# DLR-RM/AugmentedAutoencoder

Hardware: AMD Instinct MI355X
Metric: crops/sec (encode+codebook-NN), 128x128x3 vs 92232x128 codebook, 1/8 GPU (higher is better)
Workload: dtype f32; 1 GPU; configs[1]: single object per GPU, batch=256 uint8 128x128x3 crops, HIP 4-conv encoder -> 128-d + cosine-NN vs 92232x128 fp32 codebook, top-1; batch_per_gpu=256, codebook_rows=92232, latent=128, parallelism=single GPU

## Files before the change

### augmentedautoencoder_amd/csrc/aae_abi_impl.h

```cpp
#pragma once

extern "C" {

int aae_abi_version(void) { return AAE_ABI_VERSION; }
const char* aae_last_error(void) { return aae_host::g_last_error.c_str(); }

int aae_encoder_create(const aae_encoder_desc* d, const void* const* hw, int n_weights, aae_encoder** out) {
    using namespace aae_host;
    if (!d || !hw || !out) return fail(AAE_ERR_INVALID, "aae_encoder_create: null argument");
    if (d->num_layers < 1 || d->num_layers > AAE_MAX_LAYERS)
        return fail(AAE_ERR_INVALID, "num_layers %d outside [1,%d]", d->num_layers, AAE_MAX_LAYERS);
    if (d->in_h < 1 || d->in_w < 1 || d->in_c < 1 || d->kernel_size < 1 || d->latent_size < 1)
        return fail(AAE_ERR_INVALID, "non-positive shape in encoder desc");
    const int per_layer = d->batch_norm ? 6 : 2;
    if (n_weights != d->num_layers * per_layer + 2)
        return fail(AAE_ERR_INVALID, "expected %d weight arrays, got %d", d->num_layers * per_layer + 2, n_weights);
    for (int i = 0; i < n_weights; ++i)
        if (!hw[i]) return fail(AAE_ERR_INVALID, "weight array %d is null", i);

    aae_encoder* enc = new aae_encoder();
    enc->desc = *d;
    auto bail = [&](int rc) { aae_encoder_destroy(enc); return rc; };

    {
// ... 251 lines not shown
        if (value < -8 || value > 12) return fail(AAE_ERR_INVALID, "x3h_act_shift %d outside [-8, 12]", value);
        enc->x3h_act_shift = value;
    } else if (!strcmp(name, "winograd")) {
        if (value != 0) {
            bool any = false;
            for (const Layer& L : enc->layers) any = any || L.wino_geom >= 0;
            if (!any) return fail(AAE_ERR_UNSUPPORTED, "winograd: no layer is eligible (5 x 5 stride-2 'SAME' layers behind the first one with 32 | Cin, 64 | Cout and 16 | Ho, Wo or an 8 x 8 output)");
        }
        if (value < 0 || value > 2) return fail(AAE_ERR_INVALID, "winograd %d: 0 = direct kernels, 1 = one launch per layer, 2 = one launch per polyphase component", value);
#ifndef AAE_EXPERIMENTS
        if (value == 2) return fail(AAE_ERR_UNSUPPORTED, "option 'winograd' = 2 (one launch per polyphase component: measured slower) is a kernel variant of the experiments build (-DAAE_EXPERIMENTS)");
#endif
        enc->winograd = value;
    } else if (!strcmp(name, "winograd_wide")) {
        enc->winograd_wide = value ? 1 : 0;
    } else if (!strcmp(name, "winograd_min_batch")) {
        enc->winograd_min_batch = value < 1 ? 1 : value;
    } else if (!strcmp(name, "winograd_min_fill_pct")) {
        enc->winograd_min_fill_pct = value < 1 ? 1 : (value > 100 ? 100 : value);
    } else if (!strcmp(name, "winograd_min_blocks")) {
        enc->winograd_min_blocks = value < 0 ? 0 : value;
    } else if (!strcmp(name, "multi_mid_group")) {
        enc->multi_mid_group = value ? 1 : 0;
    } else if (!strcmp(name, "multi_split_items")) {
        enc->multi_split_items = value ? 1 : 0;
    } else if (!strcmp(name, "multi_group_winograd")) {
        enc->multi_group_winograd = value ? 1 : 0;
    } else if (!strcmp(name, "multi_mid_scan")) {
        enc->multi_mid_scan = value ? 1 : 0;
    } else if (!strcmp(name, "multi_mid_ragged")) {
// ... 458 lines not shown
```

### augmentedautoencoder_amd/csrc/aae_encoder_launch.h

```cpp
#pragma once

namespace aae_host {

struct Timer {
    bool on = false;
    hipStream_t stream = nullptr;
    std::vector<hipEvent_t> ev;
    int mark() {
        if (!on) return AAE_OK;
        hipEvent_t e;
        AAE_HIP_TRY(hipEventCreate(&e));
        ev.push_back(e);
        AAE_HIP_TRY(hipEventRecord(e, stream));
        return AAE_OK;
    }
};

static int launch_igemm(aae_encoder* enc, const Layer& L, const float* x, int M, float* out, float* partial,
                        hipStream_t stream, Timer& tm, const char* name, int tag = 0) {
    aae::ConvIgemmArgs a;
    a.x = x; a.wp = L.wp; a.bias = L.bias; a.bn_scale = L.bn_scale; a.bn_shift = L.bn_shift;
    a.H = L.H; a.W = L.W; a.Cin = L.Cin; a.Ho = L.Ho; a.Wo = L.Wo; a.Cout = L.Cout; a.CoutPad = L.CoutPad;
    a.KS = L.KS; a.S = L.S; a.pt = L.pt; a.pl = L.pl; a.M = M; a.relu = L.relu; a.stagger = enc->igemm_stagger;
    const unsigned long long x_bytes = (unsigned long long)(M / (L.Ho * L.Wo)) * L.H * L.W * L.Cin * sizeof(float);
// ... 520 lines not shown
            if (L.wino_geom == 0) launch_wino_phase<0>(a, eh, ew, grid, stream);
            else launch_wino_phase<1>(a, eh, ew, grid, stream);
            const int taps = (eh ? 3 : 2) * (ew ? 3 : 2), points = ((eh ? 3 : 2) + 1) * ((ew ? 3 : 2) + 1);
            snprintf(label, sizeof(label), "%s:conv_wino_f32 phase %d%d (%d taps as %d products per 2x2 outputs) M=%d N=%d C=%d", name, eh, ew, taps, points,
                     B * L.Ho * L.Wo, L.Cout, L.Cin);
            note_kernel({label, 2.0 * tiles * points * (double)L.Cin * (double)L.Cout});
            AAE_HIP_TRY(hipGetLastError());
            if (int rc = tm.mark()) return rc;
        }
        return AAE_OK;
    }
#endif
    aae::ConvWinoLayerArgs p;
    p.c = a;
    for (int i = 0; i < 4; ++i) p.U4[i] = L.wino[i];
    wino_layer_launch(L.wino_geom, enc->winograd_wide, grid, stream, p);
    snprintf(label, sizeof(label), "%s:conv_wino_f32 layer (25 taps as 49 products per 2x2 outputs) M=%d N=%d C=%d", name, B * L.Ho * L.Wo, L.Cout, L.Cin);
    note_kernel({label, 2.0 * tiles * 49.0 * (double)L.Cin * (double)L.Cout});
    AAE_HIP_TRY(hipGetLastError());
    return tm.mark();
}

static bool winograd_rule(const aae_encoder* enc, const Layer& L, int B);
static bool runs_winograd(const aae_encoder* enc, const Layer& L, int B) { return L.wino[0] && winograd_rule(enc, L, B); }
static bool wants_winograd_weights(const aae_encoder* enc, int B) {
    for (const Layer& L : enc->layers)
        if (L.kind == KIND_IGEMM && !L.wino[0] && winograd_rule(enc, L, B)) return true;
    return false;
}
static int ensure_winograd_weights(aae_encoder* enc) {
    std::lock_guard<std::mutex> lk(enc->wino_mu);
// ... 184 lines not shown
```

### augmentedautoencoder_amd/csrc/aae_host_types.h

```cpp
#pragma once

namespace aae_host {

static thread_local std::string g_last_error;

static int fail(int code, const char* fmt, ...) {
    char buf[512];
    va_list ap;
    va_start(ap, fmt);
    vsnprintf(buf, sizeof(buf), fmt, ap);
    va_end(ap);
    g_last_error = buf;
    return code;
}

#define AAE_HIP_TRY(expr)                                                                       \
    do {                                                                                        \
        hipError_t e__ = (expr);                                                                \
        if (e__ != hipSuccess)                                                                  \
            return aae_host::fail(AAE_ERR_RUNTIME, "%s failed: %s (%s:%d)", #expr,              \
                                  hipGetErrorString(e__), __FILE__, __LINE__);                  \
    } while (0)

static inline size_t align_up(size_t v, size_t a) { return (v + a - 1) / a * a; }
// ... 57 lines not shown
    std::mutex rec_mu;
    int splitk_min_base_blocks = 384;
    int splitk_target_blocks = 512;
    int reduce_small = 1;
    int precision = 0;
    int winograd = 1;
    int winograd_wide = 0;
    int winograd_min_batch = 8;
    int winograd_min_fill_pct = 56;
    int winograd_min_blocks = 0;
    int multi_mid_group = 1;
    int multi_split_items = 1;
    int multi_group_winograd = 1;
    int multi_mid_scan = 1;
    int multi_mid_ragged = 1;
    int winograd_xcd_cols = -1;
    int first_target_blocks = 512;
    int first_group_split_max_tiles = 128;
    int first_vec4 = 1;
    int first_max_tiles_per_block = 16;
    int igemm_breg_min_blocks = 768;
    int igemm_breg_wide = 1;
    int igemm_breg_wide_min_blocks = 512;
    int dense_gemv = 1;
    int dense_gemv_max_batch = 8;
    int igemm_breg = 1;
    int igemm_dma = 1;
    int x3h_wide_min_blocks = 0;
    int x3h_wide256 = 1;
    int x3h_wide256_min_blocks = 256;
// ... 57 lines not shown
```

### augmentedautoencoder_amd/csrc/aae_multi_impl.h

```cpp
#pragma once

namespace aae_host {

struct MultiItemPlan {
    bool grouped = false;
    bool mid = false;
    int n = 0, row0 = 0;
    size_t enc_off = 0, enc_bytes = 0, cb_off = 0, cb_bytes = 0;
    Workspace ws;
    std::vector<WaveKPlan> plans;
    std::vector<WaveKPlan> rem_plans;
    size_t rem_partial_off = 0, rem_partial_bytes = 0;
    ScanPlan sp;
    const aae_codebook* eff = nullptr;
    int idx_scale = 1;
    std::vector<int> sig;
};

struct MultiPlan {
    std::vector<MultiItemPlan> items;
    std::vector<std::vector<int>> groups;
    std::vector<std::vector<int>> mid_groups;
    std::vector<std::vector<char>> group_wino;
    std::vector<std::vector<char>> mid_wino;
// ... 540 lines not shown
            wm.range.n = (int)members.size();
            for (size_t k = 0; k < members.size(); ++k) {
                const MultiItemPlan& p = mp.items[(size_t)members[k]];
                const Layer& L = items[members[k]].enc->layers[li];
                aae::ConvWinoObject& ob = wm.obj[k];
                ob.x = reinterpret_cast<const float*>(enc_base(k) + p.ws.act_off[li - 1]);
                ob.out = reinterpret_cast<float*>(enc_base(k) + p.ws.act_off[li]);
                for (int q = 0; q < 4; ++q) ob.U4[q] = L.wino[q];
                ob.bias = L.bias; ob.bn_scale = L.bn_scale; ob.bn_shift = L.bn_shift; ob.B = p.n;
                wm.range.first[k] = wat;
                wat += wino_regions(L, p.n);
            }
            wm.range.first[members.size()] = wat;
            c.regions = wat;
            c.xcd_cols = wino_xcd_cols(enc0, L0);
            wino_layer_multi_launch(L0.wino_geom, aae::wino_grid_blocks(wat, L0.Cout / 64, c.xcd_cols), stream, wm);
            AAE_HIP_TRY(hipGetLastError());
            ++t_multi_launches;
            continue;
        }
        aae::ConvWaveKMultiArgs m;
        memset(&m, 0, sizeof(m));
        m.range.n = (int)members.size();
        int at = 0;
        for (size_t k = 0; k < members.size(); ++k) {
            const aae_multi_item& it = items[members[k]];
            const MultiItemPlan& p = mp.items[(size_t)members[k]];
            const Layer& L = it.enc->layers[li];
            const WaveKPlan& w = p.plans[li];
            m.item[k] = wavek_args(it.enc, L, w, reinterpret_cast<const float*>(enc_base(k) + p.ws.act_off[li - 1]), p.n * L.Ho * L.Wo,
                                   reinterpret_cast<float*>(enc_base(k) + p.ws.act_off[li]), reinterpret_cast<float*>(enc_base(k) + p.ws.partial_off),
// ... 128 lines not shown
        for (size_t k = 0; k < members.size(); ++k) {
            const MultiItemPlan& p = mp.items[(size_t)members[k]];
            const Layer& L = items[members[k]].enc->layers[li];
            aae::ConvWinoObject& ob = m.obj[k];
            ob.x = reinterpret_cast<const float*>(base + p.enc_off + p.ws.act_off[li - 1]);
            ob.out = reinterpret_cast<float*>(base + p.enc_off + p.ws.act_off[li]);
            for (int q = 0; q < 4; ++q) ob.U4[q] = L.wino[q];
            ob.bias = L.bias; ob.bn_scale = L.bn_scale; ob.bn_shift = L.bn_shift;
            ob.B = split ? p.n / 4 * 4 : p.n;
            m.range.first[k] = at;
            at += wino_regions(L, ob.B);
        }
        m.range.first[members.size()] = at;
        c.regions = at;
        c.xcd_cols = wino_xcd_cols(enc0, L0);
        wino_layer_multi_launch(L0.wino_geom, aae::wino_grid_blocks(at, L0.Cout / 64, c.xcd_cols), stream, m);
        AAE_HIP_TRY(hipGetLastError());
        ++t_multi_launches;
        if (split) {
            aae::ConvWaveKMultiArgs r;
            memset(&r, 0, sizeof(r));
            const unsigned nonce = next_nonce();
            int rat = 0, nk = 0;
            const WaveKPlan* w0 = nullptr;
            for (size_t k = 0; k < members.size(); ++k) {
                const aae_multi_item& it = items[members[k]];
                const MultiItemPlan& p = mp.items[(size_t)members[k]];
                const Layer& L = it.enc->layers[li];
                const WaveKPlan& w = p.rem_plans[li];
                const int full = p.n / 4 * 4, rem = p.n - full;
                if (!rem || !w.use) continue;
// ... 270 lines not shown
```

### augmentedautoencoder_amd/csrc/aae_wino_launch.h

```cpp
#pragma once

namespace aae_host {

#ifdef AAE_WINO_DECLARATIONS_ONLY
void wino_layer_launch(int geom, int wide, unsigned grid, hipStream_t stream, const aae::ConvWinoLayerArgs& p);
void wino_layer_multi_launch(int geom, unsigned grid, hipStream_t stream, const aae::ConvWinoMultiArgs& p);
void wino_set_attributes();
#else
#ifdef AAE_WINO_TU
#define AAE_WINO_LINKAGE
#else
#define AAE_WINO_LINKAGE static
#endif
AAE_WINO_LINKAGE void wino_layer_launch(int geom, int wide, unsigned grid, hipStream_t stream, const aae::ConvWinoLayerArgs& p) {
#ifdef AAE_EXPERIMENTS
    if (wide) {
        if (geom == 0) AAE_LAUNCH((aae::conv_wino_layer_kernel<0, true>), dim3(grid), dim3(256), aae::wino_layer_smem_bytes<0>(), stream, p);
        else AAE_LAUNCH((aae::conv_wino_layer_kernel<1, true>), dim3(grid), dim3(256), aae::wino_layer_smem_bytes<1>(), stream, p);
        return;
    }
#endif
    (void)wide;
    if (geom == 0) AAE_LAUNCH((aae::conv_wino_layer_kernel<0, false>), dim3(grid), dim3(512), aae::wino_layer_smem_bytes<0>(), stream, p);
    else AAE_LAUNCH((aae::conv_wino_layer_kernel<1, false>), dim3(grid), dim3(512), aae::wino_layer_smem_bytes<1>(), stream, p);
}
AAE_WINO_LINKAGE void wino_layer_multi_launch(int geom, unsigned grid, hipStream_t stream, const aae::ConvWinoMultiArgs& p) {
    if (geom == 0) AAE_LAUNCH((aae::conv_wino_layer_multi_kernel<0>), dim3(grid), dim3(512), aae::wino_layer_smem_bytes<0>(), stream, p);
    else AAE_LAUNCH((aae::conv_wino_layer_multi_kernel<1>), dim3(grid), dim3(512), aae::wino_layer_smem_bytes<1>(), stream, p);
}
AAE_WINO_LINKAGE void wino_set_attributes() {
    (void)hipFuncSetAttribute((const void*)aae::conv_wino_layer_multi_kernel<0>, hipFuncAttributeMaxDynamicSharedMemorySize, aae::wino_layer_smem_bytes<0>());
    (void)hipFuncSetAttribute((const void*)aae::conv_wino_layer_multi_kernel<1>, hipFuncAttributeMaxDynamicSharedMemorySize, aae::wino_layer_smem_bytes<1>());
    (void)hipFuncSetAttribute((const void*)aae::conv_wino_layer_kernel<0, false>, hipFuncAttributeMaxDynamicSharedMemorySize, aae::wino_layer_smem_bytes<0>());
    (void)hipFuncSetAttribute((const void*)aae::conv_wino_layer_kernel<1, false>, hipFuncAttributeMaxDynamicSharedMemorySize, aae::wino_layer_smem_bytes<1>());
#ifdef AAE_EXPERIMENTS
    (void)hipFuncSetAttribute((const void*)aae::conv_wino_layer_kernel<0, true>, hipFuncAttributeMaxDynamicSharedMemorySize, aae::wino_layer_smem_bytes<0>());
    (void)hipFuncSetAttribute((const void*)aae::conv_wino_layer_kernel<1, true>, hipFuncAttributeMaxDynamicSharedMemorySize, aae::wino_layer_smem_bytes<1>());
#endif
}
#endif

}
```

### augmentedautoencoder_amd/csrc/kernels/conv_winograd_f32.h

```cpp
#pragma once
#include <type_traits>

#include "multi_launch.h"

namespace aae {

struct ConvWinoArgs {
    const float* x;
    const float* U;
    const float* bias;
    const float* bn_scale;
    const float* bn_shift;
    float* out;
    int B, H, W, Cin, Cout, Ho, Wo;
    int eh, ew;
    int mode;
    int relu;
    int blocks_x, blocks_y;
    int regions;
    int xcd_cols;
#ifdef AAE_WINO_STAMPS
    long long* stamps;
#endif
};
// ... 4 lines not shown
#define AAE_WINO_STAMP(a, slot) do {} while (0)
#endif
inline unsigned wino_grid_blocks(int regions, int nbn, int xcd_cols) {
    if (xcd_cols <= 0) return (unsigned)regions * (unsigned)nbn;
    const int region_groups = 8 / (nbn / xcd_cols);
    return 8u * (unsigned)xcd_cols * (unsigned)((regions + region_groups - 1) / region_groups);
}
inline bool wino_xcd_cols_valid(int nbn, int xcd_cols) {
    return xcd_cols >= 1 && nbn % xcd_cols == 0 && (nbn / xcd_cols) <= 8 && 8 % (nbn / xcd_cols) == 0;
}

template <int GEOM>
struct WinoGeom;
template <>
struct WinoGeom<0> {
    static constexpr int kImages = 1, kRows = 18, kCols = 18, kRowPitch = 12, kParityPitch = 220, kImagePitch = 2 * 220;
};
template <>
struct WinoGeom<1> {
    static constexpr int kImages = 4, kRows = 10, kCols = 10, kRowPitch = 6, kParityPitch = 60, kImagePitch = 128;
};
template <int GEOM>
constexpr int wino_plane_units() { return WinoGeom<GEOM>::kImages * WinoGeom<GEOM>::kImagePitch + 1; }
template <int GEOM>
constexpr int wino_stage_units() { return 8 * wino_plane_units<GEOM>(); }
template <int GEOM>
constexpr int wino_smem_bytes() { return 2 * wino_stage_units<GEOM>() * 16; }

struct ConvWinoLayerArgs {
    ConvWinoArgs c;
    const float* U4[4];
};
struct ConvWinoObject {
    const float* x;
    float* out;
    const float* U4[4];
    const float* bias;
    const float* bn_scale;
    const float* bn_shift;
    int B, pad_;
};
struct ConvWinoMultiArgs {
    ConvWinoArgs c;
    MultiRange range;
    ConvWinoObject obj[kMultiMax];
};
template <int GEOM>
constexpr int wino_layer_stage_bytes() { return 2 * 4 * wino_plane_units<GEOM>() * 16; }
template <int GEOM>
constexpr int wino_layer_smem_bytes() { return wino_layer_stage_bytes<GEOM>() + 4 * 64 * 64 * 4; }


#ifndef AAE_WINO_DECLARATIONS_ONLY

#if defined(__HIP_DEVICE_COMPILE__)
__device__ __forceinline__ f32x2 wino_pk_add(f32x2 a, f32x2 b) {
    f32x2 r;
    asm("v_pk_add_f32 %0, %1, %2" : "=v"(r) : "v"(a), "v"(b));
    return r;
}
__device__ __forceinline__ f32x2 wino_pk_sub(f32x2 a, f32x2 b) {
    f32x2 r;
    asm("v_pk_add_f32 %0, %1, %2 neg_lo:[0,1] neg_hi:[0,1]" : "=v"(r) : "v"(a), "v"(b));
    return r;
}
// ... 33 lines not shown
__device__ __forceinline__ float wino_sub1(float a, float b) {
    float r;
    asm("v_sub_f32 %0, %1, %2" : "=v"(r) : "v"(a), "v"(b));
    return r;
}
__device__ __forceinline__ float wino_nadd1(float a, float b) {
    float r;
    asm("v_sub_f32 %0, -%1, %2" : "=v"(r) : "v"(a), "v"(b));
    return r;
}
#else
__host__ __device__ inline float wino_add1(float a, float b) { return a + b; }
__host__ __device__ inline float wino_sub1(float a, float b) { return a - b; }
__host__ __device__ inline float wino_nadd1(float a, float b) { return -a - b; }
#endif
template <int N>
__device__ __forceinline__ void wino_acc_fence(f32x16 (&c)[N]) {
#if defined(__HIP_DEVICE_COMPILE__)
    static_assert(N == 6 || N == 8, "2 PB accumulator tiles");
    if constexpr (N == 8)
        asm volatile("s_nop 15\n\ts_nop 3" : "+v"(c[0]), "+v"(c[1]), "+v"(c[2]), "+v"(c[3]), "+v"(c[4]), "+v"(c[5]), "+v"(c[6]), "+v"(c[7]));
    else
        asm volatile("s_nop 15\n\ts_nop 3" : "+v"(c[0]), "+v"(c[1]), "+v"(c[2]), "+v"(c[3]), "+v"(c[4]), "+v"(c[5]));
#else
    (void)c;
#endif
}

struct WinoBlock {
    int nb, region, img0, wy0, wx0;
    bool live;
};
__device__ __forceinline__ void wino_block_index(int block, int nbn, int regions, int xcd_cols, WinoBlock& w) {
    if (xcd_cols > 0) {
        const int col_groups = nbn / xcd_cols, region_groups = 8 / col_groups, chunk = (regions + region_groups - 1) / region_groups;
        const int xcd = block & 7, within = block >> 3, k = within / xcd_cols;
        w.nb = (xcd % col_groups) * xcd_cols + within % xcd_cols;
        w.region = (xcd / col_groups) * chunk + k;
// ... 16 lines not shown
        w.wx0 = 16 * bx - 1;
    } else {
        w.img0 = 4 * local;
        w.wy0 = w.wx0 = -1;
    }
}
template <int GEOM>
__device__ __forceinline__ WinoBlock wino_block(int block, int nbn, int blocks_x, int blocks_y, int regions, int xcd_cols) {
    WinoBlock w;
    wino_block_index(block, nbn, regions, xcd_cols, w);
    wino_block_geometry<GEOM>(w.region, blocks_x, blocks_y, w);
    return w;
}
template <int GEOM>
__device__ __forceinline__ void wino_tile(int mh, int t, int& ti, int& ty, int& tx) {
    if (GEOM == 0) { ti = 0; ty = 4 * mh + (t >> 3); tx = t & 7; }
    else { ti = 2 * mh + (t >> 4); ty = (t >> 2) & 3; tx = t & 3; }
}



template <int GEOM, int STAGE_CH, int NT>
struct WinoFillPlan {
    static constexpr int kQuads = STAGE_CH / 4, kParts = STAGE_CH / 16;
    static constexpr int kStageQuads = WinoGeom<GEOM>::kImages * WinoGeom<GEOM>::kRows * WinoGeom<GEOM>::kCols * kQuads;
    static constexpr int kPer = ((kStageQuads + NT - 1) / NT + kParts - 1) / kParts;
    uint32_t goff[kParts * kPer];
    int lslot[kParts * kPer];
};
constexpr uint32_t kWinoOutside = 0x80000000u;
template <int GEOM, int STAGE_CH, int NT>
__device__ __forceinline__ void wino_fill_plan(const ConvWinoArgs& a, const WinoBlock& wb, WinoFillPlan<GEOM, STAGE_CH, NT>& f) {
    using G = WinoGeom<GEOM>;
    using F = WinoFillPlan<GEOM, STAGE_CH, NT>;
    constexpr int kPlane = wino_plane_units<GEOM>();
    const int cq_per_pixel = a.Cin / 4;
#pragma unroll
    for (int i = 0; i < F::kParts * F::kPer; ++i) {
        const int idx = (int)threadIdx.x + NT * i;
        f.goff[i] = kWinoOutside;
        f.lslot[i] = -1;
        if (idx < F::kStageQuads) {
            const int pixel = idx / F::kQuads, cq = idx - pixel * F::kQuads;
            const int wi = pixel / (G::kRows * G::kCols), rem = pixel - wi * (G::kRows * G::kCols);
            const int wy = rem / G::kCols, wx = rem - wy * G::kCols;
            const int uu = wb.wy0 + wy, vv = wb.wx0 + wx, b = wb.img0 + wi;
            if (uu >= 0 && uu < a.Ho && vv >= 0 && vv < a.Wo && b < a.B)
                f.goff[i] = (uint32_t)(((((size_t)b * a.H + 2 * uu) * a.W + 2 * vv) * cq_per_pixel + cq) * 16);
            f.lslot[i] = cq * kPlane + wi * G::kImagePitch + (wx & 1) * G::kParityPitch + wy * G::kRowPitch + (wx >> 1);
        }
    }
}

template <int TA, int TB, bool SWAP, int GEOM, int STAGE_CH, bool ACCUMULATE, bool WIDE, int CHAIN = 0, int NTA = 3, int NTB = 3>
__device__ __forceinline__ void wino_phase_body(const ConvWinoArgs& a, const float* U, int eh, int ew, const WinoBlock& wb, f32x4* lds, float* xch_all,
                                                const WinoFillPlan<GEOM, STAGE_CH, WIDE ? 256 : 512>& fill, int& buf0, f32x4 (&uin)[8],
                                                const float* Un, int neh, int new_, f32x4 (&uout)[8]) {
    using G = WinoGeom<GEOM>;
    using F = WinoFillPlan<GEOM, STAGE_CH, WIDE ? 256 : 512>;
    constexpr int PB = TB + 1;
    constexpr int kQuads = STAGE_CH / 4, kGroups = STAGE_CH / 8;
    constexpr int kPlane = wino_plane_units<GEOM>(), kStage = kQuads * kPlane;
    constexpr int kParity = G::kParityPitch;
    constexpr int kParts = F::kParts, kPer = F::kPer;
    constexpr int NH = WIDE ? 2 : 1;
    constexpr int kOffA = TA == 2 ? 1 : 0, kOffB = TB == 2 ? 1 : 0;
// ... 3 lines not shown
    int li, lty, ltx;
    wino_tile<GEOM>(mh, m, li, lty, ltx);
    const int n32 = wb.nb * 2 + nh, KG = a.Cin / 8, nst = a.Cin / STAGE_CH;
    constexpr int NP = (TA + 1) * PB;
    constexpr int kPhaseNo = TA == 3 && TB == 3 ? 0 : (TA == 3 && !SWAP ? 1 : (TA == 3 ? 2 : 3));
    (void)kPhaseNo;
    AAE_WINO_STAMP(a, 4 * kPhaseNo + 0);
    const buffer_rsrc xrs = make_buffer(a.x, (uint32_t)((size_t)a.B * a.H * a.W * a.Cin * 4));
    const buffer_rsrc urs = make_buffer(U, (uint32_t)((size_t)NP * a.Cin * a.Cout * 4));
    const uint32_t ulane = (uint32_t)(((size_t)n32 * KG * NP + (size_t)ph * 2 * PB) * 64 + h * 32 + m) * 16u;
    const bool two_rows = TA == 3 || ph == 0;
    const uint32_t parity_off = (uint32_t)(((size_t)eh * a.W + ew) * a.Cin * 4);
    const uint32_t next_parity_off = (uint32_t)(((size_t)neh * a.W + new_) * a.Cin * 4);

    f32x16 acc[NH][2 * PB];
#pragma unroll
    for (int n2 = 0; n2 < NH; ++n2)
#pragma unroll
        for (int p = 0; p < 2 * PB; ++p)
#pragma unroll
            for (int r = 0; r < 16; ++r) acc[n2][p][r] = 0.f;

    f32x4 stg[kPer];
    auto stage_load = [&](uint32_t soff, int part) {
#pragma unroll
        for (int i = 0; i < kPer; ++i) stg[i] = buffer_load4_s(xrs, fill.goff[part * kPer + i], soff);
    };
    auto stage_store = [&](int buf, int part) {
#pragma unroll
        for (int i = 0; i < kPer; ++i)
            if (fill.lslot[part * kPer + i] >= 0) lds[buf * kStage + fill.lslot[part * kPer + i]] = stg[i];
    };
    auto fA = [](int pos) { return SWAP ? (pos & 1) * kParity + (pos >> 1) : pos * G::kRowPitch; };
    auto fB = [](int pos) { return SWAP ? pos * G::kRowPitch : (pos & 1) * kParity + (pos >> 1); };
    const int lane_base = li * G::kImagePitch + 2 * lty * G::kRowPitch + ltx;
    const int posA0 = (TA == 3 ? (ph == 0 ? 0 : 2) : (ph == 0 ? 0 : 1)) + kOffA;
    const int posA1 = (ph == 0 ? 1 : 3) + kOffA;
    const int posA2 = (TA == 3 ? (ph == 0 ? 2 : 1) : (ph == 0 ? 1 : 2)) + kOffA;
    const int offA0 = fA(posA0), offA1 = fA(posA1), offA2 = fA(posA2);
    const float sg = ph == 0 ? 1.f : -1.f;

    const uint32_t half_stride = (uint32_t)KG * NP * 1024u;
    f32x4 u[NH][2 * PB];
    if (CHAIN & 1) {
#pragma unroll
        for (int p = 0; p < 2 * PB; ++p) u[0][p] = uin[p];
// ... 33 lines not shown
        if (TB == 3) {
            const f32x4 e0 = w[0], e1 = w[1], e2 = w[2], e3 = w[PB - 1];
            w[0] = wino_sub4(e0, e2);
            w[1] = wino_add4(e1, e2);
            w[2] = wino_sub4(e2, e1);
            w[PB - 1] = wino_sub4(e1, e3);
        } else {
            const f32x4 e0 = w[0], e1 = w[1], e2 = w[2];
            w[0] = wino_sub4(e0, e1);
            w[2] = wino_sub4(e1, e2);
        }
    };
    auto run = [&](auto rows_tag) {
        constexpr int ROWS = decltype(rows_tag)::value, NU = kGroups * ROWS, kPartUnits = NU / kParts;
        static_assert(NU % 2 == 0 && NU % kParts == 0, "units per stage");
        constexpr int kStoreBack = (kParts == 1 && NU >= 4) ? 2 : 1;
        const bool early = ph == 1 && NU >= 4 && kParts == 1;
        f32x4 raw[2 * PB], v[PB];
        read_unit(lds + buf0 * kStage + h * kPlane + lane_base, 0, raw);
        for (int st = 0; st < nst; ++st) {
            const int buf = (buf0 + st) & 1;
            const bool more = st + 1 < nst;
            const bool filling = more || (CHAIN & 2);
            const uint32_t fill_off = more ? parity_off + (uint32_t)(st + 1) * kQuads * 16 : next_parity_off;
#ifdef AAE_WINO_STAMPS
            if (kPhaseNo == 0 && st < 8) AAE_WINO_STAMP(a, 20 + st);
#endif
            const f32x4* stage = lds + buf * kStage + h * kPlane + lane_base;
            const f32x4* next_stage = lds + (buf ^ 1) * kStage + h * kPlane + lane_base;
#pragma unroll
            for (int t = 0; t < NU; ++t) {
                const int i = t % ROWS, slot = t & 1;
#ifdef AAE_WINO_STAMPS
                if (kPhaseNo == 0 && (st == 2 || st == 3) && t < 4) AAE_WINO_STAMP(a, 28 + 6 * (st - 2) + t);
#endif
                step_a(i, raw, v);
                step_b(v);
                if ((st > 0 || t > 0) && (more || t + 1 < NU)) {
                    const int tn = (t + 1) % NU, gn = (st + (t + 1) / NU) * kGroups + tn / ROWS;
                    const uint32_t un = (uint32_t)gn * (NP * 1024u) + (tn % ROWS) * PB * 1024u;
#pragma unroll
                    for (int n2 = 0; n2 < NH; ++n2)
#pragma unroll
                        for (int j = 0; j < PB; ++j) u[n2][(slot ^ 1) * PB + j] = buffer_load4_s(urs, ulane + j * 1024u, un + n2 * half_stride);
                }
                if (filling && t % kPartUnits == 0) stage_load(fill_off, t / kPartUnits);
                if (filling && t % kPartUnits == kPartUnits - kStoreBack) stage_store(buf ^ 1, t / kPartUnits);
                if (t + 1 < NU) read_unit(stage + 2 * ((t + 1) / ROWS) * kPlane, (t + 1) % ROWS, raw);
                if (filling && (t == NU - 1 ? !early : (t == NU - 2 && early))) {
#ifdef AAE_WINO_STAMPS
                    if (kPhaseNo == 0 && (st == 2 || st == 3)) AAE_WINO_STAMP(a, 28 + 6 * (st - 2) + 4);
#endif
                    __syncthreads();
#ifdef AAE_WINO_STAMPS
                    if (kPhaseNo == 0 && (st == 2 || st == 3)) AAE_WINO_STAMP(a, 28 + 6 * (st - 2) + 5);
#endif
                }
                if (t == NU - 1 && more) read_unit(next_stage, 0, raw);
                sched_fence();
#pragma unroll
                for (int q = 0; q < 4; ++q)
#pragma unroll
                    for (int j = 0; j < PB; ++j)
#pragma unroll
                        for (int n2 = 0; n2 < NH; ++n2)
                            acc[n2][(ROWS == 2 ? i * PB : 0) + j] = mfma_32x32x2(v[j][q], u[n2][slot * PB + j][q], acc[n2][(ROWS == 2 ? i * PB : 0) + j]);
                sched_fence();
            }
        }
    };
    if (TA == 3 || ph == 0) run(std::integral_constant<int, 2>());
    else run(std::integral_constant<int, 1>());
    if (STAGE_CH == 32 && !(CHAIN & 2)) __syncthreads();
    AAE_WINO_STAMP(a, 4 * kPhaseNo + 2);
    if (CHAIN & 2) {
        constexpr int NPB = NTB + 1, NNP = (NTA + 1) * NPB;
        const buffer_rsrc nrs = make_buffer(Un, (uint32_t)((size_t)NNP * a.Cin * a.Cout * 4));
        const uint32_t nlane = (uint32_t)(((size_t)n32 * KG * NNP + (size_t)ph * 2 * NPB) * 64 + h * 32 + m) * 16u;
        const bool next_two_rows = NTA == 3 || ph == 0;
#pragma unroll
        for (int p = 0; p < 2 * NPB; ++p)
            uout[p] = buffer_load4_s(nrs, nlane + (p % NPB) * 1024u, next_two_rows ? (p / NPB) * NPB * 1024u : (p / NPB) * (NNP * 1024u));
    }
    buf0 = (buf0 + nst) & 1;
#pragma unroll
    for (int n2 = 0; n2 < NH; ++n2) wino_acc_fence(acc[n2]);

    auto drain = [&](auto ph_tag) {
        constexpr int PH = decltype(ph_tag)::value;
        auto partial = [&](int n2, int r, float (&y)[4]) {
            constexpr bool kNoQ0 = PH == 1 && TA == 2;
            float q0[PB], q1[PB];
#pragma unroll
            for (int j = 0; j < PB; ++j) {
                const float mA = acc[n2][j][r], mB = acc[n2][PB + j][r];
                if (PH == 0) { q0[j] = wino_add1(mA, mB); q1[j] = mB; }
                else if (TA == 3) { q0[j] = mA; q1[j] = wino_nadd1(mA, mB); }
                else { q0[j] = 0.f; q1[j] = -mA; }
            }
            float t[4];
            if (TB == 3) {
                t[0] = kNoQ0 ? 0.f : wino_add1(wino_add1(q0[0], q0[1]), q0[2]);
                t[1] = kNoQ0 ? 0.f : wino_sub1(wino_sub1(q0[1], q0[2]), q0[3]);
                t[2] = wino_add1(wino_add1(q1[0], q1[1]), q1[2]);
                t[3] = wino_sub1(wino_sub1(q1[1], q1[2]), q1[3]);
            } else {
                t[0] = kNoQ0 ? 0.f : wino_add1(q0[0], q0[1]);
                t[1] = kNoQ0 ? 0.f : wino_sub1(q0[1], q0[2]);
                t[2] = wino_add1(q1[0], q1[1]);
                t[3] = wino_sub1(q1[1], q1[2]);
// ... 100 lines not shown
template <int TA, int TB, bool SWAP, int GEOM>
__global__ __launch_bounds__(512) void conv_wino_phase_kernel(ConvWinoArgs a) {
    AAE_DYN_SMEM(smem_raw);
    const WinoBlock wb = wino_block<GEOM>(blockIdx.x, a.Cout / 64, a.blocks_x, a.blocks_y, a.regions, a.xcd_cols);
    if (!wb.live) return;
    WinoFillPlan<GEOM, 32, 512> fill;
    wino_fill_plan(a, wb, fill);
    int buf0 = 0;
    f32x4 unused[8];
    wino_phase_body<TA, TB, SWAP, GEOM, 32, false, false>(a, a.U, a.eh, a.ew, wb, reinterpret_cast<f32x4*>(smem_raw), reinterpret_cast<float*>(smem_raw), fill, buf0, unused,
                                                          nullptr, 0, 0, unused);
    wino_store_block<GEOM, 512>(a, a.mode, wb, reinterpret_cast<const float*>(smem_raw));
}
#endif

template <int GEOM, bool WIDE>
__device__ __forceinline__ void wino_layer_block(const ConvWinoArgs& a, const float* const (&U4)[4], const WinoBlock& wb, unsigned char* smem_raw) {
    f32x4* lds = reinterpret_cast<f32x4*>(smem_raw);
    float* xch = reinterpret_cast<float*>(smem_raw + wino_layer_stage_bytes<GEOM>());
    WinoFillPlan<GEOM, 16, WIDE ? 256 : 512> fill;
    wino_fill_plan(a, wb, fill);
    int buf0 = 0;
    f32x4 ua[8], ub[8];
    if (WIDE) {
        wino_phase_body<3, 3, false, GEOM, 16, false, WIDE>(a, U4[3], 1, 1, wb, lds, xch, fill, buf0, ua, nullptr, 0, 0, ub);
        wino_phase_body<3, 2, false, GEOM, 16, true, WIDE>(a, U4[2], 1, 0, wb, lds, xch, fill, buf0, ua, nullptr, 0, 0, ub);
        wino_phase_body<3, 2, true, GEOM, 16, true, WIDE>(a, U4[1], 0, 1, wb, lds, xch, fill, buf0, ua, nullptr, 0, 0, ub);
        wino_phase_body<2, 2, false, GEOM, 16, true, WIDE>(a, U4[0], 0, 0, wb, lds, xch, fill, buf0, ua, nullptr, 0, 0, ub);
    } else {
        constexpr bool W = WIDE;
        wino_phase_body<3, 3, false, GEOM, 16, false, W, W ? 0 : 2, 3, 2>(a, U4[3], 1, 1, wb, lds, xch, fill, buf0, ua, U4[2], 1, 0, ub);
        wino_phase_body<3, 2, false, GEOM, 16, true, W, W ? 0 : 3, 3, 2>(a, U4[2], 1, 0, wb, lds, xch, fill, buf0, ub, U4[1], 0, 1, ua);
        wino_phase_body<3, 2, true, GEOM, 16, true, W, W ? 0 : 3, 2, 2>(a, U4[1], 0, 1, wb, lds, xch, fill, buf0, ua, U4[0], 0, 0, ub);
        wino_phase_body<2, 2, false, GEOM, 16, true, W, W ? 0 : 1>(a, U4[0], 0, 0, wb, lds, xch, fill, buf0, ub, nullptr, 0, 0, ua);
    }
    wino_store_block<GEOM, WIDE ? 256 : 512>(a, 3, wb, xch);
}

template <int GEOM, bool WIDE>
__global__ __launch_bounds__(WIDE ? 256 : 512) void conv_wino_layer_kernel(ConvWinoLayerArgs p) {
    AAE_DYN_SMEM(smem_raw);
    const ConvWinoArgs& a = p.c;
    const WinoBlock wb = wino_block<GEOM>(blockIdx.x, a.Cout / 64, a.blocks_x, a.blocks_y, a.regions, a.xcd_cols);
    if (!wb.live) return;
    wino_layer_block<GEOM, WIDE>(a, p.U4, wb, smem_raw);
#ifdef AAE_WINO_STAMPS
    asm volatile("s_waitcnt vmcnt(0)" ::: "memory");
    AAE_WINO_STAMP(a, 16);
    if (threadIdx.x == 0) a.stamps[((size_t)blockIdx.x * 8) * kWinoStampSlots + 17] = (long long)(__builtin_amdgcn_s_getreg(20 | (0 << 6) | (3 << 11)) & 15);
#endif
}

template <int GEOM>
__global__ __launch_bounds__(512) void conv_wino_layer_multi_kernel(ConvWinoMultiArgs p) {
    AAE_DYN_SMEM(smem_raw);
    WinoBlock wb;
    wino_block_index(blockIdx.x, p.c.Cout / 64, p.c.regions, p.c.xcd_cols, wb);
    if (!wb.live) return;
    const int o = multi_find(p.range, wb.region);
    wino_block_geometry<GEOM>(wb.region - p.range.first[o], p.c.blocks_x, p.c.blocks_y, wb);
    ConvWinoArgs a = p.c;
    const ConvWinoObject& ob = p.obj[o];
    a.x = ob.x; a.out = ob.out; a.bias = ob.bias; a.bn_scale = ob.bn_scale; a.bn_shift = ob.bn_shift; a.B = ob.B;
    const float* U4[4] = {ob.U4[0], ob.U4[1], ob.U4[2], ob.U4[3]};
    wino_layer_block<GEOM, false>(a, U4, wb, smem_raw);
}

#endif

}
```

Baseline: 55850 crops/s.

## Stage 32 channels per Winograd LDS buffer and prefetch first stage and fragments

```diff
diff --git a/augmentedautoencoder_amd/csrc/aae_abi_impl.h b/augmentedautoencoder_amd/csrc/aae_abi_impl.h
--- a/augmentedautoencoder_amd/csrc/aae_abi_impl.h
+++ b/augmentedautoencoder_amd/csrc/aae_abi_impl.h
@@ -289,6 +289,8 @@
         enc->winograd = value;
     } else if (!strcmp(name, "winograd_wide")) {
         enc->winograd_wide = value ? 1 : 0;
+    } else if (!strcmp(name, "winograd_stage32")) {
+        enc->winograd_stage32 = value ? 1 : 0;
     } else if (!strcmp(name, "winograd_min_batch")) {
         enc->winograd_min_batch = value < 1 ? 1 : value;
     } else if (!strcmp(name, "winograd_min_fill_pct")) {
diff --git a/augmentedautoencoder_amd/csrc/aae_encoder_launch.h b/augmentedautoencoder_amd/csrc/aae_encoder_launch.h
--- a/augmentedautoencoder_amd/csrc/aae_encoder_launch.h
+++ b/augmentedautoencoder_amd/csrc/aae_encoder_launch.h
@@ -558,7 +558,7 @@
     aae::ConvWinoLayerArgs p;
     p.c = a;
     for (int i = 0; i < 4; ++i) p.U4[i] = L.wino[i];
-    wino_layer_launch(L.wino_geom, enc->winograd_wide, grid, stream, p);
+    wino_layer_launch(L.wino_geom, enc->winograd_wide, enc->winograd_stage32, grid, stream, p);
     snprintf(label, sizeof(label), "%s:conv_wino_f32 layer (25 taps as 49 products per 2x2 outputs) M=%d N=%d C=%d", name, B * L.Ho * L.Wo, L.Cout, L.Cin);
     note_kernel({label, 2.0 * tiles * 49.0 * (double)L.Cin * (double)L.Cout});
     AAE_HIP_TRY(hipGetLastError());
diff --git a/augmentedautoencoder_amd/csrc/aae_host_types.h b/augmentedautoencoder_amd/csrc/aae_host_types.h
--- a/augmentedautoencoder_amd/csrc/aae_host_types.h
+++ b/augmentedautoencoder_amd/csrc/aae_host_types.h
@@ -95,6 +95,7 @@
     int multi_group_winograd = 1;
     int multi_mid_scan = 1;
     int multi_mid_ragged = 1;
+    int winograd_stage32 = 1;
     int winograd_xcd_cols = -1;
     int first_target_blocks = 512;
     int first_group_split_max_tiles = 128;
diff --git a/augmentedautoencoder_amd/csrc/aae_multi_impl.h b/augmentedautoencoder_amd/csrc/aae_multi_impl.h
--- a/augmentedautoencoder_amd/csrc/aae_multi_impl.h
+++ b/augmentedautoencoder_amd/csrc/aae_multi_impl.h
@@ -578,7 +578,7 @@
             wm.range.first[members.size()] = wat;
             c.regions = wat;
             c.xcd_cols = wino_xcd_cols(enc0, L0);
-            wino_layer_multi_launch(L0.wino_geom, aae::wino_grid_blocks(wat, L0.Cout / 64, c.xcd_cols), stream, wm);
+            wino_layer_multi_launch(L0.wino_geom, enc0->winograd_stage32, aae::wino_grid_blocks(wat, L0.Cout / 64, c.xcd_cols), stream, wm);
             AAE_HIP_TRY(hipGetLastError());
             ++t_multi_launches;
             continue;
@@ -737,7 +737,7 @@
         m.range.first[members.size()] = at;
         c.regions = at;
         c.xcd_cols = wino_xcd_cols(enc0, L0);
-        wino_layer_multi_launch(L0.wino_geom, aae::wino_grid_blocks(at, L0.Cout / 64, c.xcd_cols), stream, m);
+        wino_layer_multi_launch(L0.wino_geom, enc0->winograd_stage32, aae::wino_grid_blocks(at, L0.Cout / 64, c.xcd_cols), stream, m);
         AAE_HIP_TRY(hipGetLastError());
         ++t_multi_launches;
         if (split) {
diff --git a/augmentedautoencoder_amd/csrc/aae_wino_launch.h b/augmentedautoencoder_amd/csrc/aae_wino_launch.h
--- a/augmentedautoencoder_amd/csrc/aae_wino_launch.h
+++ b/augmentedautoencoder_amd/csrc/aae_wino_launch.h
@@ -3,8 +3,8 @@
 namespace aae_host {
 
 #ifdef AAE_WINO_DECLARATIONS_ONLY
-void wino_layer_launch(int geom, int wide, unsigned grid, hipStream_t stream, const aae::ConvWinoLayerArgs& p);
-void wino_layer_multi_launch(int geom, unsigned grid, hipStream_t stream, const aae::ConvWinoMultiArgs& p);
+void wino_layer_launch(int geom, int wide, int stage32, unsigned grid, hipStream_t stream, const aae::ConvWinoLayerArgs& p);
+void wino_layer_multi_launch(int geom, int stage32, unsigned grid, hipStream_t stream, const aae::ConvWinoMultiArgs& p);
 void wino_set_attributes();
 #else
 #ifdef AAE_WINO_TU
@@ -12,7 +12,7 @@
 #else
 #define AAE_WINO_LINKAGE static
 #endif
-AAE_WINO_LINKAGE void wino_layer_launch(int geom, int wide, unsigned grid, hipStream_t stream, const aae::ConvWinoLayerArgs& p) {
+AAE_WINO_LINKAGE void wino_layer_launch(int geom, int wide, int stage32, unsigned grid, hipStream_t stream, const aae::ConvWinoLayerArgs& p) {
 #ifdef AAE_EXPERIMENTS
     if (wide) {
         if (geom == 0) AAE_LAUNCH((aae::conv_wino_layer_kernel<0, true>), dim3(grid), dim3(256), aae::wino_layer_smem_bytes<0>(), stream, p);
@@ -21,14 +21,20 @@
     }
 #endif
     (void)wide;
-    if (geom == 0) AAE_LAUNCH((aae::conv_wino_layer_kernel<0, false>), dim3(grid), dim3(512), aae::wino_layer_smem_bytes<0>(), stream, p);
+    if (aae::wino_layer_stage_channels(geom, p.c.Cin, stage32 != 0) == 32)
+        AAE_LAUNCH((aae::conv_wino_layer_kernel<0, false, 32>), dim3(grid), dim3(512), (aae::wino_layer_smem_bytes<0, 32>()), stream, p);
+    else if (geom == 0) AAE_LAUNCH((aae::conv_wino_layer_kernel<0, false>), dim3(grid), dim3(512), aae::wino_layer_smem_bytes<0>(), stream, p);
     else AAE_LAUNCH((aae::conv_wino_layer_kernel<1, false>), dim3(grid), dim3(512), aae::wino_layer_smem_bytes<1>(), stream, p);
 }
-AAE_WINO_LINKAGE void wino_layer_multi_launch(int geom, unsigned grid, hipStream_t stream, const aae::ConvWinoMultiArgs& p) {
-    if (geom == 0) AAE_LAUNCH((aae::conv_wino_layer_multi_kernel<0>), dim3(grid), dim3(512), aae::wino_layer_smem_bytes<0>(), stream, p);
+AAE_WINO_LINKAGE void wino_layer_multi_launch(int geom, int stage32, unsigned grid, hipStream_t stream, const aae::ConvWinoMultiArgs& p) {
+    if (aae::wino_layer_stage_channels(geom, p.c.Cin, stage32 != 0) == 32)
+        AAE_LAUNCH((aae::conv_wino_layer_multi_kernel<0, 32>), dim3(grid), dim3(512), (aae::wino_layer_smem_bytes<0, 32>()), stream, p);
+    else if (geom == 0) AAE_LAUNCH((aae::conv_wino_layer_multi_kernel<0>), dim3(grid), dim3(512), aae::wino_layer_smem_bytes<0>(), stream, p);
     else AAE_LAUNCH((aae::conv_wino_layer_multi_kernel<1>), dim3(grid), dim3(512), aae::wino_layer_smem_bytes<1>(), stream, p);
 }
 AAE_WINO_LINKAGE void wino_set_attributes() {
+    (void)hipFuncSetAttribute((const void*)aae::conv_wino_layer_multi_kernel<0, 32>, hipFuncAttributeMaxDynamicSharedMemorySize, aae::wino_layer_smem_bytes<0, 32>());
+    (void)hipFuncSetAttribute((const void*)aae::conv_wino_layer_kernel<0, false, 32>, hipFuncAttributeMaxDynamicSharedMemorySize, aae::wino_layer_smem_bytes<0, 32>());
     (void)hipFuncSetAttribute((const void*)aae::conv_wino_layer_multi_kernel<0>, hipFuncAttributeMaxDynamicSharedMemorySize, aae::wino_layer_smem_bytes<0>());
     (void)hipFuncSetAttribute((const void*)aae::conv_wino_layer_multi_kernel<1>, hipFuncAttributeMaxDynamicSharedMemorySize, aae::wino_layer_smem_bytes<1>());
     (void)hipFuncSetAttribute((const void*)aae::conv_wino_layer_kernel<0, false>, hipFuncAttributeMaxDynamicSharedMemorySize, aae::wino_layer_smem_bytes<0>());
diff --git a/augmentedautoencoder_amd/csrc/kernels/conv_winograd_f32.h b/augmentedautoencoder_amd/csrc/kernels/conv_winograd_f32.h
--- a/augmentedautoencoder_amd/csrc/kernels/conv_winograd_f32.h
+++ b/augmentedautoencoder_amd/csrc/kernels/conv_winograd_f32.h
@@ -42,7 +42,7 @@
 struct WinoGeom;
 template <>
 struct WinoGeom<0> {
-    static constexpr int kImages = 1, kRows = 18, kCols = 18, kRowPitch = 12, kParityPitch = 220, kImagePitch = 2 * 220;
+    static constexpr int kImages = 1, kRows = 18, kCols = 18, kRowPitch = 10, kParityPitch = 180, kImagePitch = 2 * 180;
 };
 template <>
 struct WinoGeom<1> {
@@ -73,10 +73,12 @@
     MultiRange range;
     ConvWinoObject obj[kMultiMax];
 };
-template <int GEOM>
-constexpr int wino_layer_stage_bytes() { return 2 * 4 * wino_plane_units<GEOM>() * 16; }
-template <int GEOM>
-constexpr int wino_layer_smem_bytes() { return wino_layer_stage_bytes<GEOM>() + 4 * 64 * 64 * 4; }
+template <int GEOM, int STAGE_CH = 16>
+constexpr int wino_layer_stage_bytes() { return 2 * (STAGE_CH / 4) * wino_plane_units<GEOM>() * 16; }
+template <int GEOM, int STAGE_CH = 16>
+constexpr int wino_layer_smem_bytes() { return wino_layer_stage_bytes<GEOM, STAGE_CH>() + 4 * 64 * 64 * 4; }
+static_assert(wino_layer_smem_bytes<0, 32>() <= 160 * 1024 && wino_layer_smem_bytes<1, 16>() <= 160 * 1024, "LDS of a compute unit");
+inline int wino_layer_stage_channels(int geom, int Cin, bool stage32) { return stage32 && geom == 0 && Cin % 32 == 0 ? 32 : 16; }
 
 
 #ifndef AAE_WINO_DECLARATIONS_ONLY
@@ -140,14 +142,16 @@
 __host__ __device__ inline float wino_sub1(float a, float b) { return a - b; }
 __host__ __device__ inline float wino_nadd1(float a, float b) { return -a - b; }
 #endif
-template <int N>
-__device__ __forceinline__ void wino_acc_fence(f32x16 (&c)[N]) {
+template <int N, int M>
+__device__ __forceinline__ void wino_acc_fence(f32x16 (&c)[M]) {
 #if defined(__HIP_DEVICE_COMPILE__)
-    static_assert(N == 6 || N == 8, "2 PB accumulator tiles");
+    static_assert((N == 3 || N == 6 || N == 8) && N <= M, "PB or 2 PB accumulator tiles");
     if constexpr (N == 8)
         asm volatile("s_nop 15\n\ts_nop 3" : "+v"(c[0]), "+v"(c[1]), "+v"(c[2]), "+v"(c[3]), "+v"(c[4]), "+v"(c[5]), "+v"(c[6]), "+v"(c[7]));
+    else if constexpr (N == 6)
+        asm volatile("s_nop 15\n\ts_nop 3" : "+v"(c[0]), "+v"(c[1]), "+v"(c[2]), "+v"(c[3]), "+v"(c[4]), "+v"(c[5]));
     else
-        asm volatile("s_nop 15\n\ts_nop 3" : "+v"(c[0]), "+v"(c[1]), "+v"(c[2]), "+v"(c[3]), "+v"(c[4]), "+v"(c[5]));
+        asm volatile("s_nop 15\n\ts_nop 3" : "+v"(c[0]), "+v"(c[1]), "+v"(c[2]));
 #else
     (void)c;
 #endif
@@ -194,7 +198,7 @@
 }
 template <int GEOM>
 __device__ __forceinline__ void wino_tile(int mh, int t, int& ti, int& ty, int& tx) {
-    if (GEOM == 0) { ti = 0; ty = 4 * mh + (t >> 3); tx = t & 7; }
+    if (GEOM == 0) { const int c = t >> 2; ti = 0; ty = 4 * mh + (c >> 1); tx = 4 * ((c ^ (c >> 1) ^ (c >> 2)) & 1) + (t & 3); }
     else { ti = 2 * mh + (t >> 4); ty = (t >> 2) & 3; tx = t & 3; }
 }
 
@@ -207,6 +211,9 @@
     static constexpr int kPer = ((kStageQuads + NT - 1) / NT + kParts - 1) / kParts;
     uint32_t goff[kParts * kPer];
     int lslot[kParts * kPer];
+    __host__ __device__ static constexpr bool wave_stores(int wave, int i) { return wave * 64 + NT * i < kStageQuads; }
+    static constexpr int kSpareColumn = (WinoGeom<GEOM>::kCols + 1) / 2;
+    static_assert(kSpareColumn < WinoGeom<GEOM>::kRowPitch && 64 / kQuads <= 2 * WinoGeom<GEOM>::kRows && NT % kQuads == 0, "spare units of the stage buffer");
 };
 constexpr uint32_t kWinoOutside = 0x80000000u;
 template <int GEOM, int STAGE_CH, int NT>
@@ -215,21 +222,55 @@
     using F = WinoFillPlan<GEOM, STAGE_CH, NT>;
     constexpr int kPlane = wino_plane_units<GEOM>();
     const int cq_per_pixel = a.Cin / 4;
+    constexpr int kStep = NT / F::kQuads, kWindow = G::kRows * G::kCols;
+    constexpr int kStepI = kStep / kWindow, kStepY = kStep % kWindow / G::kCols, kStepX = kStep % G::kCols;
+    const int pixel0 = (int)threadIdx.x / F::kQuads, cq = (int)threadIdx.x % F::kQuads;
+    int wi = pixel0 / kWindow, wy = pixel0 % kWindow / G::kCols, wx = pixel0 % G::kCols;
 #pragma unroll
     for (int i = 0; i < F::kParts * F::kPer; ++i) {
         const int idx = (int)threadIdx.x + NT * i;
         f.goff[i] = kWinoOutside;
-        f.lslot[i] = -1;
         if (idx < F::kStageQuads) {
-            const int pixel = idx / F::kQuads, cq = idx - pixel * F::kQuads;
-            const int wi = pixel / (G::kRows * G::kCols), rem = pixel - wi * (G::kRows * G::kCols);
-            const int wy = rem / G::kCols, wx = rem - wy * G::kCols;
             const int uu = wb.wy0 + wy, vv = wb.wx0 + wx, b = wb.img0 + wi;
             if (uu >= 0 && uu < a.Ho && vv >= 0 && vv < a.Wo && b < a.B)
                 f.goff[i] = (uint32_t)(((((size_t)b * a.H + 2 * uu) * a.W + 2 * vv) * cq_per_pixel + cq) * 16);
             f.lslot[i] = cq * kPlane + wi * G::kImagePitch + (wx & 1) * G::kParityPitch + wy * G::kRowPitch + (wx >> 1);
-        }
-    }
+        } else {
+            const int d = (idx - F::kStageQuads) & 63, row = d / F::kQuads;
+            f.lslot[i] = cq * kPlane + (row / G::kRows) * G::kParityPitch + (row % G::kRows) * G::kRowPitch + F::kSpareColumn;
+        }
+        wx += kStepX;
+        wy += kStepY + (wx >= G::kCols ? 1 : 0);
+        wx -= wx >= G::kCols ? G::kCols : 0;
+        wi += kStepI + (wy >= G::kRows ? 1 : 0);
+        wy -= wy >= G::kRows ? G::kRows : 0;
+    }
+}
+
+template <int TA, int TB>
+__device__ __forceinline__ void wino_first_fragments(const ConvWinoArgs& a, const float* U, const WinoBlock& wb, f32x4 (&u)[8]) {
+    constexpr int PB = TB + 1, NP = (TA + 1) * PB;
+    const int tid = threadIdx.x, lane = tid & 63, wave = wave_uniform(tid >> 6);
+    const int nh = (wave >> 1) & 1, ph = wave >> 2, m = lane & 31, h = lane >> 5, n32 = wb.nb * 2 + nh, KG = a.Cin / 8;
+    const buffer_rsrc urs = make_buffer(U, (uint32_t)((size_t)NP * a.Cin * a.Cout * 4));
+    const uint32_t ulane = (uint32_t)(((size_t)n32 * KG * NP + (size_t)ph * 2 * PB) * 64 + h * 32 + m) * 16u;
+    const bool two_rows = TA == 3 || ph == 0;
+#pragma unroll
+    for (int p = 0; p < 2 * PB; ++p) u[p] = buffer_load4_s(urs, ulane + (p % PB) * 1024u, two_rows ? (p / PB) * PB * 1024u : (p / PB) * (NP * 1024u));
+}
+template <int GEOM, int STAGE_CH, int NT>
+__device__ __forceinline__ void wino_first_stage(const ConvWinoArgs& a, int eh, int ew, const WinoFillPlan<GEOM, STAGE_CH, NT>& fill, f32x4* lds) {
+    using F = WinoFillPlan<GEOM, STAGE_CH, NT>;
+    const int wave = wave_uniform((int)threadIdx.x >> 6);
+    const buffer_rsrc xrs = make_buffer(a.x, (uint32_t)((size_t)a.B * a.H * a.W * a.Cin * 4));
+    const uint32_t parity_off = (uint32_t)(((size_t)eh * a.W + ew) * a.Cin * 4);
+    f32x4 stg[F::kParts * F::kPer];
+#pragma unroll
+    for (int i = 0; i < F::kParts * F::kPer; ++i) stg[i] = buffer_load4_s(xrs, fill.goff[i], parity_off);
+#pragma unroll
+    for (int i = 0; i < F::kParts * F::kPer; ++i)
+        if (F::wave_stores(wave, i)) lds[fill.lslot[i]] = stg[i];
+    __syncthreads();
 }
 
 template <int TA, int TB, bool SWAP, int GEOM, int STAGE_CH, bool ACCUMULATE, bool WIDE, int CHAIN = 0, int NTA = 3, int NTB = 3>
@@ -263,12 +304,6 @@
     const uint32_t next_parity_off = (uint32_t)(((size_t)neh * a.W + new_) * a.Cin * 4);
 
     f32x16 acc[NH][2 * PB];
-#pragma unroll
-    for (int n2 = 0; n2 < NH; ++n2)
-#pragma unroll
-        for (int p = 0; p < 2 * PB; ++p)
-#pragma unroll
-            for (int r = 0; r < 16; ++r) acc[n2][p][r] = 0.f;
 
     f32x4 stg[kPer];
     auto stage_load = [&](uint32_t soff, int part) {
@@ -278,7 +313,7 @@
     auto stage_store = [&](int buf, int part) {
 #pragma unroll
         for (int i = 0; i < kPer; ++i)
-            if (fill.lslot[part * kPer + i] >= 0) lds[buf * kStage + fill.lslot[part * kPer + i]] = stg[i];
+            if (F::wave_stores(wave, part * kPer + i)) lds[buf * kStage + fill.lslot[part * kPer + i]] = stg[i];
     };
     auto fA = [](int pos) { return SWAP ? (pos & 1) * kParity + (pos >> 1) : pos * G::kRowPitch; };
     auto fB = [](int pos) { return SWAP ? pos * G::kRowPitch : (pos & 1) * kParity + (pos >> 1); };
@@ -342,11 +377,12 @@
     auto run = [&](auto rows_tag) {
         constexpr int ROWS = decltype(rows_tag)::value, NU = kGroups * ROWS, kPartUnits = NU / kParts;
         static_assert(NU % 2 == 0 && NU % kParts == 0, "units per stage");
-        constexpr int kStoreBack = (kParts == 1 && NU >= 4) ? 2 : 1;
-        const bool early = ph == 1 && NU >= 4 && kParts == 1;
+        constexpr int kStoreBack = kPartUnits >= 4 ? 2 : 1;
+        const bool early = ph == 1 && kStoreBack == 2;
         f32x4 raw[2 * PB], v[PB];
         read_unit(lds + buf0 * kStage + h * kPlane + lane_base, 0, raw);
-        for (int st = 0; st < nst; ++st) {
+        auto stage_body = [&](int st, auto first_tag) {
+            constexpr bool FIRST = decltype(first_tag)::value;
             const int buf = (buf0 + st) & 1;
             const bool more = st + 1 < nst;
             const bool filling = more || (CHAIN & 2);
@@ -364,7 +400,7 @@
 #endif
                 step_a(i, raw, v);
                 step_b(v);
-                if ((st > 0 || t > 0) && (more || t + 1 < NU)) {
+                if ((!FIRST || t > 0) && (more || t + 1 < NU)) {
                     const int tn = (t + 1) % NU, gn = (st + (t + 1) / NU) * kGroups + tn / ROWS;
                     const uint32_t un = (uint32_t)gn * (NP * 1024u) + (tn % ROWS) * PB * 1024u;
 #pragma unroll
@@ -391,28 +427,34 @@
 #pragma unroll
                     for (int j = 0; j < PB; ++j)
 #pragma unroll
-                        for (int n2 = 0; n2 < NH; ++n2)
-                            acc[n2][(ROWS == 2 ? i * PB : 0) + j] = mfma_32x32x2(v[j][q], u[n2][slot * PB + j][q], acc[n2][(ROWS == 2 ? i * PB : 0) + j]);
+                        for (int n2 = 0; n2 < NH; ++n2) {
+                            f32x16& c = acc[n2][(ROWS == 2 ? i * PB : 0) + j];
+                            if (FIRST && t < ROWS && q == 0) c = mfma_32x32x2(v[j][q], u[n2][slot * PB + j][q], f32x16{});
+                            else c = mfma_32x32x2(v[j][q], u[n2][slot * PB + j][q], c);
+                        }
                 sched_fence();
             }
-        }
+        };
+        stage_body(0, std::true_type());
+        for (int st = 1; st < nst; ++st) stage_body(st, std::false_type());
     };
     if (TA == 3 || ph == 0) run(std::integral_constant<int, 2>());
     else run(std::integral_constant<int, 1>());
-    if (STAGE_CH == 32 && !(CHAIN & 2)) __syncthreads();
+    if (STAGE_CH == 32 && CHAIN == 0) __syncthreads();
     AAE_WINO_STAMP(a, 4 * kPhaseNo + 2);
     if (CHAIN & 2) {
-        constexpr int NPB = NTB + 1, NNP = (NTA + 1) * NPB;
-        const buffer_rsrc nrs = make_buffer(Un, (uint32_t)((size_t)NNP * a.Cin * a.Cout * 4));
-        const uint32_t nlane = (uint32_t)(((size_t)n32 * KG * NNP + (size_t)ph * 2 * NPB) * 64 + h * 32 + m) * 16u;
-        const bool next_two_rows = NTA == 3 || ph == 0;
-#pragma unroll
-        for (int p = 0; p < 2 * NPB; ++p)
-            uout[p] = buffer_load4_s(nrs, nlane + (p % NPB) * 1024u, next_two_rows ? (p / NPB) * NPB * 1024u : (p / NPB) * (NNP * 1024u));
+        wino_first_fragments<NTA, NTB>(a, Un, wb, uout);
     }
     buf0 = (buf0 + nst) & 1;
 #pragma unroll
-    for (int n2 = 0; n2 < NH; ++n2) wino_acc_fence(acc[n2]);
+    for (int n2 = 0; n2 < NH; ++n2) {
+        if constexpr (TA == 2) {
+            if (ph == 1) wino_acc_fence<PB>(acc[n2]);
+            else wino_acc_fence<2 * PB>(acc[n2]);
+        } else {
+            wino_acc_fence<2 * PB>(acc[n2]);
+        }
+    }
 
     auto drain = [&](auto ph_tag) {
         constexpr int PH = decltype(ph_tag)::value;
@@ -421,7 +463,7 @@
             float q0[PB], q1[PB];
 #pragma unroll
             for (int j = 0; j < PB; ++j) {
-                const float mA = acc[n2][j][r], mB = acc[n2][PB + j][r];
+                const float mA = acc[n2][j][r], mB = kNoQ0 ? 0.f : acc[n2][PB + j][r];
                 if (PH == 0) { q0[j] = wino_add1(mA, mB); q1[j] = mB; }
                 else if (TA == 3) { q0[j] = mA; q1[j] = wino_nadd1(mA, mB); }
                 else { q0[j] = 0.f; q1[j] = -mA; }
@@ -552,36 +594,40 @@
 }
 #endif
 
-template <int GEOM, bool WIDE>
+template <int GEOM, bool WIDE, int STAGE_CH>
 __device__ __forceinline__ void wino_layer_block(const ConvWinoArgs& a, const float* const (&U4)[4], const WinoBlock& wb, unsigned char* smem_raw) {
+    constexpr int SC = STAGE_CH;
+    static_assert(SC == 16 || (SC == 32 && !WIDE), "stage size");
     f32x4* lds = reinterpret_cast<f32x4*>(smem_raw);
-    float* xch = reinterpret_cast<float*>(smem_raw + wino_layer_stage_bytes<GEOM>());
-    WinoFillPlan<GEOM, 16, WIDE ? 256 : 512> fill;
-    wino_fill_plan(a, wb, fill);
+    float* xch = reinterpret_cast<float*>(smem_raw + wino_layer_stage_bytes<GEOM, SC>());
+    WinoFillPlan<GEOM, SC, WIDE ? 256 : 512> fill;
     int buf0 = 0;
     f32x4 ua[8], ub[8];
+    if (!WIDE) wino_first_fragments<3, 3>(a, U4[3], wb, ua);
+    wino_fill_plan(a, wb, fill);
     if (WIDE) {
-        wino_phase_body<3, 3, false, GEOM, 16, false, WIDE>(a, U4[3], 1, 1, wb, lds, xch, fill, buf0, ua, nullptr, 0, 0, ub);
-        wino_phase_body<3, 2, false, GEOM, 16, true, WIDE>(a, U4[2], 1, 0, wb, lds, xch, fill, buf0, ua, nullptr, 0, 0, ub);
-        wino_phase_body<3, 2, true, GEOM, 16, true, WIDE>(a, U4[1], 0, 1, wb, lds, xch, fill, buf0, ua, nullptr, 0, 0, ub);
-        wino_phase_body<2, 2, false, GEOM, 16, true, WIDE>(a, U4[0], 0, 0, wb, lds, xch, fill, buf0, ua, nullptr, 0, 0, ub);
+        wino_phase_body<3, 3, false, GEOM, SC, false, WIDE>(a, U4[3], 1, 1, wb, lds, xch, fill, buf0, ua, nullptr, 0, 0, ub);
+        wino_phase_body<3, 2, false, GEOM, SC, true, WIDE>(a, U4[2], 1, 0, wb, lds, xch, fill, buf0, ua, nullptr, 0, 0, ub);
+        wino_phase_body<3, 2, true, GEOM, SC, true, WIDE>(a, U4[1], 0, 1, wb, lds, xch, fill, buf0, ua, nullptr, 0, 0, ub);
+        wino_phase_body<2, 2, false, GEOM, SC, true, WIDE>(a, U4[0], 0, 0, wb, lds, xch, fill, buf0, ua, nullptr, 0, 0, ub);
     } else {
         constexpr bool W = WIDE;
-        wino_phase_body<3, 3, false, GEOM, 16, false, W, W ? 0 : 2, 3, 2>(a, U4[3], 1, 1, wb, lds, xch, fill, buf0, ua, U4[2], 1, 0, ub);
-        wino_phase_body<3, 2, false, GEOM, 16, true, W, W ? 0 : 3, 3, 2>(a, U4[2], 1, 0, wb, lds, xch, fill, buf0, ub, U4[1], 0, 1, ua);
-        wino_phase_body<3, 2, true, GEOM, 16, true, W, W ? 0 : 3, 2, 2>(a, U4[1], 0, 1, wb, lds, xch, fill, buf0, ua, U4[0], 0, 0, ub);
-        wino_phase_body<2, 2, false, GEOM, 16, true, W, W ? 0 : 1>(a, U4[0], 0, 0, wb, lds, xch, fill, buf0, ub, nullptr, 0, 0, ua);
+        if (!W) wino_first_stage(a, 1, 1, fill, lds);
+        wino_phase_body<3, 3, false, GEOM, SC, false, W, W ? 0 : 3, 3, 2>(a, U4[3], 1, 1, wb, lds, xch, fill, buf0, ua, U4[2], 1, 0, ub);
+        wino_phase_body<3, 2, false, GEOM, SC, true, W, W ? 0 : 3, 3, 2>(a, U4[2], 1, 0, wb, lds, xch, fill, buf0, ub, U4[1], 0, 1, ua);
+        wino_phase_body<3, 2, true, GEOM, SC, true, W, W ? 0 : 3, 2, 2>(a, U4[1], 0, 1, wb, lds, xch, fill, buf0, ua, U4[0], 0, 0, ub);
+        wino_phase_body<2, 2, false, GEOM, SC, true, W, W ? 0 : 1>(a, U4[0], 0, 0, wb, lds, xch, fill, buf0, ub, nullptr, 0, 0, ua);
     }
     wino_store_block<GEOM, WIDE ? 256 : 512>(a, 3, wb, xch);
 }
 
-template <int GEOM, bool WIDE>
+template <int GEOM, bool WIDE, int STAGE_CH = 16>
 __global__ __launch_bounds__(WIDE ? 256 : 512) void conv_wino_layer_kernel(ConvWinoLayerArgs p) {
     AAE_DYN_SMEM(smem_raw);
     const ConvWinoArgs& a = p.c;
     const WinoBlock wb = wino_block<GEOM>(blockIdx.x, a.Cout / 64, a.blocks_x, a.blocks_y, a.regions, a.xcd_cols);
     if (!wb.live) return;
-    wino_layer_block<GEOM, WIDE>(a, p.U4, wb, smem_raw);
+    wino_layer_block<GEOM, WIDE, STAGE_CH>(a, p.U4, wb, smem_raw);
 #ifdef AAE_WINO_STAMPS
     asm volatile("s_waitcnt vmcnt(0)" ::: "memory");
     AAE_WINO_STAMP(a, 16);
@@ -589,7 +635,7 @@
 #endif
 }
 
-template <int GEOM>
+template <int GEOM, int STAGE_CH = 16>
 __global__ __launch_bounds__(512) void conv_wino_layer_multi_kernel(ConvWinoMultiArgs p) {
     AAE_DYN_SMEM(smem_raw);
     WinoBlock wb;
@@ -601,9 +647,9 @@
     const ConvWinoObject& ob = p.obj[o];
     a.x = ob.x; a.out = ob.out; a.bias = ob.bias; a.bn_scale = ob.bn_scale; a.bn_shift = ob.bn_shift; a.B = ob.B;
     const float* U4[4] = {ob.U4[0], ob.U4[1], ob.U4[2], ob.U4[3]};
-    wino_layer_block<GEOM, false>(a, U4, wb, smem_raw);
-}
-
-#endif
-
-}
+    wino_layer_block<GEOM, false, STAGE_CH>(a, U4, wb, smem_raw);
+}
+
+#endif
+
+}
```

New measurement: 57520 crops/s, median of 6. 3.0% higher.
